# orting/image-feature-extraction

Hardware: AMD Instinct MI355X
Metric: Mvoxels/sec Hessian+eig, 512^3 fp32 3-scale (higher is better)
Workload: dtype f32 storage / f64 line recurrences

## Files before the change

### image-feature-extraction_amd/csrc/ife_capi.hip

```cpp
#include "../../include/ife_hip.h"

#include <hip/hip_runtime.h>

#include <algorithm>
#include <cmath>
#include <cstdarg>
#include <cstdio>
#include <cstdlib>
#include <cstring>
#include <map>
#include <new>
#include <string>
#include <tuple>
#include <type_traits>
#include <vector>

#include "feature_kernels.hpp"
#include "iir_types.hpp"
#include "stats_kernels.hpp"
#include "distance_kernels.hpp"
#include "dense_kernels.hpp"
#include "dense_plan.hpp"
#include "labels_kernels.hpp"
#include "deflate_kernels.hpp"
#include "resample_kernels.hpp"
#include "bspline_kernels.hpp"
#define IFE_IIR_NS iir_exact
#define IFE_IIR_FMA 0
#include "iir_kernels.inc"
#undef IFE_IIR_NS
#undef IFE_IIR_FMA
#define IFE_IIR_NS iir_fma
#define IFE_IIR_FMA 1
#include "iir_kernels.inc"
#undef IFE_IIR_NS
#undef IFE_IIR_FMA

using namespace ife;

namespace {

#define IFE_IIR_KERNELS(NS)                                                                      \
  struct NS##_kernels {                                                                          \
    template <int K> static constexpr auto contig = NS::iir_contig_kernel<K>;                    \
    template <int K> static constexpr auto strided1 = NS::iir_strided1_kernel<K>;                \
    template <int K, bool PAIRED, bool BWD> static constexpr auto strided = NS::iir_strided_kernel<K, PAIRED, BWD>; \
    template <int K, int S, typename TI, typename TM> static constexpr auto sweep_z = NS::iir_sweep_z_kernel<K, S, TI, TM>; \
    template <int K> static constexpr auto zslab_causal = NS::zslab_causal_kernel<K>;            \
    template <int K> static constexpr auto zslab_anti = NS::zslab_anti_kernel<K>;                \
    template <int K> static constexpr auto zslab_causal3 = NS::zslab_causal3_kernel<K>;          \
    template <int K> static constexpr auto zslab_anti3 = NS::zslab_anti3_kernel<K>;              \
    template <int K, int DIR> static constexpr auto zslab_fused = NS::zslab_fused_kernel<K, DIR>; \
    template <int K> static constexpr auto zslab_combine = NS::zslab_combine_kernel<K>;          \
  }
IFE_IIR_KERNELS(iir_exact);
IFE_IIR_KERNELS(iir_fma);
#undef IFE_IIR_KERNELS
template <typename F>
void with_iir_kernels(int fma, F &&f) {
  if (fma) f(iir_fma_kernels{});
  else f(iir_exact_kernels{});
}

template <int V0, int... Vs, typename F>
void with_const(int v, F &&f) {
  if constexpr (sizeof...(Vs) == 0) f(std::integral_constant<int, V0>{});
  else if (v == V0) f(std::integral_constant<int, V0>{});
  else with_const<Vs...>(v, f);
}

enum KernelKind {
  KK_IIR_Z = 0,
  KK_IIR_X,
  KK_IIR_Y,
  KK_ZSLAB_SWEEP,
  KK_ZSLAB_COMBINE,
  KK_FEATURES,
  KK_EIG_BATCH,
  KK_DIVIDE,
  KK_MASK,
  KK_PREP,
  KK_SORT_HIST,
  KK_SORT_SCAN,
  KK_SORT_SCATTER,
  KK_GATHER,
  KK_EDGES,
  KK_HIST,
  KK_EDT_X,
  KK_EDT_Y,
  KK_EDT_Z,
  KK_EDT_REDUCE,
  KK_DENSE_CODE,
  KK_DENSE_XY,
  KK_DENSE_Z,
  KK_JET,
  KK_COUNT
};
static_assert(KK_COUNT <= IFE_MAX_KERNEL_KINDS, "ife_get_kernel_times callers size their arrays by IFE_MAX_KERNEL_KINDS");
const char *kKindNames[KK_COUNT] = {"iir_z", "iir_x", "iir_y", "zslab_sweep", "zslab_combine", "features", "eig_batch",
                                    "divide", "mask_f64", "prep", "sort_hist", "sort_scan",
                                    "sort_scatter", "gather", "edges", "dense_histogram", "edt_x", "edt_y",
                                    "edt_z", "edt_reduce", "dense_code", "dense_box_xy", "dense_box_z", "jet_features"};

struct DevBuf {
  void *p = nullptr;
  size_t cap = 0;
  DevBuf() = default;
  DevBuf(DevBuf &&o) noexcept : p(std::exchange(o.p, nullptr)), cap(std::exchange(o.cap, 0)) {}
  DevBuf &operator=(DevBuf &&o) noexcept { std::swap(p, o.p); std::swap(cap, o.cap); return *this; }
  ~DevBuf() { (void)reset(); }
  hipError_t reset() {
    cap = 0;
    return p ? hipFree(std::exchange(p, nullptr)) : hipSuccess;
  }
  hipError_t grow(size_t bytes) {
    hipError_t e = reset();
    if (e == hipSuccess && (e = hipMalloc(&p, bytes)) == hipSuccess) cap = bytes;
    else p = nullptr;
    return e;
  }
};
constexpr int IFE_MAX_SLOTS = 3;

struct ProfRec {
  int kind;
  hipEvent_t a, b;
};

thread_local std::string g_create_error;

}

struct ife_ctx {
  int device = 0;
  hipStream_t stream = nullptr;
  std::string err;
  int trig_mode = 2;
  int dscale_mode = 0;
  int profile = 0;
  int zchunk = 64;
  int iir_block = 0;
  int iir_fma = 0;
  int iir_ckpt = 2;
  int fused_divide = 1;
  int const_lines = 1;
  int feat_ring = 1;
  int z_sweep = 1;
  int differential = 0;
  std::map<std::tuple<double, double, int64_t>, uint32_t> const_flags;
  DevBuf fld[IFE_MAX_SLOTS][4];
  DevBuf pre[2];
  DevBuf ck_y[IIR_MAX_JOBS];
  DevBuf zs_rec;
  DevBuf st_img, st_mask, st_aux, st_out;
  DevBuf edt_g, edt_i, edt_d2, edt_part;
  DevBuf dn_centres, dn_ws, dn_feat;
  int dense_scratch_mb = 0;
  struct DenseStream {
    bool open = false;
    DevBuf codes;
    DevBuf centres;
    DevBuf ws;
    DevBuf planar;
    DevBuf rows[2];
    hipEvent_t done[2] = {nullptr, nullptr};
    hipStream_t copy = nullptr;
    std::vector<DenseBlock> blocks;
    size_t next = 0, counted = 0;
    DenseGeom g;
    const uint8_t *flag = nullptr;
    const uint32_t *seg_base = nullptr;
    int ncol = 0, nb = 0, values = 0, cg = 0, bg = 0;
    int64_t n_rois = 0, ld = 0;
  } ds;
  DevBuf dj_ws;
  DevBuf sc_out;
  std::vector<hipEvent_t> sc_done;
  hipStream_t sc_copy = nullptr;
  size_t sc_scale_bytes = 0;
  int sc_layout = IFE_INTERLEAVED;
  DevBuf df_ws, df_out;
  DevBuf rs_tab;
  std::vector<ResampleEntry> rs_host;
  hipEvent_t rs_up = nullptr;
  DevBuf bs_coef, bs_tab;
  std::vector<double> bs_host;
  hipEvent_t bs_up = nullptr;
  std::vector<ProfRec> prof;
  std::vector<hipEvent_t> ev_pool;
  double acc_ms[KK_COUNT] = {0};
  int64_t acc_n[KK_COUNT] = {0};
};

namespace {

void dense_stream_release(ife_ctx *ctx);

int fail(ife_ctx *ctx, int code, const char *fmt, ...) {
  char buf[512];
// ... 231 lines not shown
    const double s2 = dscale_mode == 1 ? s1 * s1 : s1;
    d.m1[a] = -0.5 * s1;
    d.p1[a] = 0.5 * s1;
    d.a2[a] = 1.0 * s2;
    d.b2[a] = -2.0 * s2;
    d.c2[a] = 1.0 * s2;
  }
  return d;
}

IirGeom geom_for_axis(const ife_volume_desc *v, int axis) {
  IirGeom g;
  g.in_w = 0; g.in_group = 0; g.in_nz = 0;
  const int64_t nx = v->nx, ny = v->ny, nz = v->nz;
  if (axis == 2) {
    g.n = nz; g.nlines = nx * ny; g.sstride = nx * ny; g.inner = nx * ny; g.outer = 0;
  } else if (axis == 1) {
    g.n = ny; g.nlines = nx * nz; g.sstride = nx; g.inner = nx; g.outer = nx * ny;
  } else {
    g.n = nx; g.nlines = ny * nz; g.sstride = 1; g.inner = 1; g.outer = nx;
  }
  return g;
}

size_t ck_pairs(int64_t n, int K) { return (size_t)((n + K - 1) / K); }

int ensure_ck(ife_ctx *ctx, const ife_volume_desc *v, int njobs) {
  const int K = 8;
  size_t need_y = 0;
  for (int a = 0; a < 3; ++a) {
    IirGeom g = geom_for_axis(v, a);
    const size_t np = ck_pairs(g.n, K);
    need_y = std::max(need_y, np * 4 * (size_t)g.nlines * sizeof(double));
  }
  for (int j = 0; j < njobs; ++j) {
    int rc = ensure(ctx, ctx->ck_y[j], need_y);
    if (rc) return rc;
  }
  return IFE_OK;
}

int ensure_slots(ife_ctx *ctx, const ife_volume_desc *v, int nslots) {
  const size_t nb = (size_t)(v->nx * v->ny * v->nz) * sizeof(float);
  for (int s = 0; s < nslots; ++s)
    for (int i = 0; i < 4; ++i) {
      int rc = ensure(ctx, ctx->fld[s][i], nb);
      if (rc) return rc;
    }
  return IFE_OK;
}

struct ZSweepSrc {
  const void *img, *msk;
  int img_dtype, msk_dtype;
  float *tc, *cf;
  int nf;
  bool write_src;
};
int launch_iir(ife_ctx *ctx, const ife_volume_desc *v, int axis, int njobs,
               const float *const *in, float *const *out, const double *sigma,
               int in_y_chunks = 1, const int *order = nullptr ,
               const float *const *in2 = nullptr, const ZSweepSrc *zs = nullptr) {
  if (njobs < 1 || njobs > IIR_MAX_JOBS) return fail(ctx, IFE_E_ARG, "bad job count %d", njobs);
  IirGeom g = geom_for_axis(v, axis);
  if (in_y_chunks > 1) {
    if (axis != 0) return fail(ctx, IFE_E_ARG, "Y-chunked input is only read by the x pass");
    if (v->ny % in_y_chunks || (v->ny / in_y_chunks) % 64)
      return fail(ctx, IFE_E_SIZE, "Y-chunked input needs ny/chunks to be a multiple of 64");
    g.in_w = in_y_chunks;
    g.in_group = v->ny / in_y_chunks;
    g.in_nz = v->nz;
  }
  if ((int64_t)2 * 16 * g.sstride * 4 >= (int64_t)1 << 31 ||
      g.outer * 4 >= (int64_t)1 << 32 || g.nlines * 8 * 3 >= (int64_t)1 << 32)
    return fail(ctx, IFE_E_SIZE, "volume too large for the 32-bit offsets of the line kernels");
  if (in2 && (axis == 0 || 2 * njobs > IIR_MAX_JOBS || ctx->iir_ckpt != 2))
    return fail(ctx, IFE_E_ARG, "the paired form runs on the strided axes with at most %d jobs", IIR_MAX_JOBS / 2);
  if (zs && (axis != 2 || in2 || order || ctx->iir_ckpt != 2 || zs->nf < 1 || zs->nf > 2 || njobs % zs->nf ||
             njobs / zs->nf > IFE_MAX_SLOTS || !zs->img || !zs->tc || (zs->nf == 2 && (!zs->msk || !zs->cf))))
    return fail(ctx, IFE_E_ARG, "the shared sweep runs the Z pass of up to %d scales with pair checkpoints", IFE_MAX_SLOTS);
  int rc = ensure_ck(ctx, v, in2 ? 2 * njobs : njobs);
  if (rc) return rc;
  if (zs && (rc = ensure(ctx, ctx->zs_rec, (size_t)zs->nf * (size_t)g.nlines * sizeof(uint32_t)))) return rc;
  uint32_t any_const = 0;
  const double sp = axis == 0 ? v->sx : axis == 1 ? v->sy : v->sz;
  IirJobs jobs;
  memset(&jobs, 0, sizeof jobs);
  for (int j = 0; j < njobs; ++j) {
    if (!in[j] || !out[j] || in[j] == out[j]) return fail(ctx, IFE_E_ARG, "bad job buffers");
    if ((reinterpret_cast<uintptr_t>(in[j]) | reinterpret_cast<uintptr_t>(out[j])) % 4)
      return fail(ctx, IFE_E_ARG, "field pointers must be aligned to 4 bytes");
    jobs.j[j].in = in[j];
    jobs.j[j].out = out[j];
    jobs.j[j].ck_y = (double *)ctx->ck_y[j].p;
    if (in2) {
      if (!in2[j] || in2[j] == out[j] || reinterpret_cast<uintptr_t>(in2[j]) % 4)
        return fail(ctx, IFE_E_ARG, "bad denominator buffer");
      jobs.j[j].in2 = in2[j];
      jobs.j[j].ck_y2 = (double *)ctx->ck_y[njobs + j].p;
    }
    if (gauss_coeffs_order(sigma[j], sp, order ? order[j] : 0, &jobs.j[j].c))
      return fail(ctx, IFE_E_ARG, "spacing is suspiciously small");
    jobs.j[j].const_lines = 0;
    if (ctx->const_lines && !ctx->iir_fma && (!order || order[j] == 0)) {
      const int64_t len = axis == 0 ? v->nx : axis == 1 ? v->ny : v->nz;
      const std::tuple<double, double, int64_t> key(sigma[j], sp, len);
      auto it = ctx->const_flags.find(key);
      if (it == ctx->const_flags.end()) {
        if (ctx->const_flags.size() > 256) ctx->const_flags.clear();
        it = ctx->const_flags.emplace(key, const_line_flags(jobs.j[j].c, len)).first;
      }
      jobs.j[j].const_lines = it->second;
    }
    any_const |= jobs.j[j].const_lines;
    if (zs) jobs.j[j].line_rec = (const uint32_t *)ctx->zs_rec.p + (size_t)(j % zs->nf) * (size_t)g.nlines;
  }
  g.njobs = njobs;
  g.ngroups = (int32_t)((g.nlines + (in2 ? 127 : 255)) / (in2 ? 128 : 256));
  const dim3 grid((unsigned)((g.ngroups + 7) / 8 * 8 * njobs), 1, 1);
  const int sblock = ctx->iir_block ? ctx->iir_block : 12;
  if (zs) {
    ProfScope pz(ctx, KK_PREP);
    ZSweepArgs za;
    za.img = zs->img; za.msk = zs->msk; za.tc = zs->tc; za.cf = zs->cf;
    za.rec = (uint32_t *)ctx->zs_rec.p;
    za.nf = zs->nf; za.write_src = zs->write_src ? 1 : 0; za.track = any_const ? 1 : 0;
    IirGeom gs = g;
    gs.njobs = zs->nf;
    const dim3 sgrid((unsigned)((gs.ngroups + 7) / 8 * 8 * zs->nf), 1, 1);
    with_iir_kernels(ctx->iir_fma, [&](auto ks) {
      using KS = decltype(ks);
      with_const<8, 10, 12, 16>(sblock, [&](auto K) {
        with_const<1, 2, 3>(njobs / zs->nf, [&](auto S) {
          auto launch = [&](auto ti, auto tm) {
            hipLaunchKernelGGL((KS::template sweep_z<decltype(K)::value, decltype(S)::value, decltype(ti), decltype(tm)>),
                               sgrid, dim3(256), 0, ctx->stream, jobs, gs, za);
          };
          auto with_mask = [&](auto ti) {
            if (zs->msk && zs->msk_dtype == IFE_U16) launch(ti, uint16_t{});
            else launch(ti, uint8_t{});
          };
          if (zs->img_dtype == IFE_F32) with_mask(float{});
          else with_mask(int16_t{});
        });
      });
    });
    IFE_HIP(ctx, hipGetLastError());
  }
  ProfScope ps(ctx, axis == 2 ? KK_IIR_Z : axis == 1 ? KK_IIR_Y : KK_IIR_X);
  with_iir_kernels(ctx->iir_fma, [&](auto ks) {
    using KS = decltype(ks);
    auto launch = [&](auto kernel) { hipLaunchKernelGGL(kernel, grid, dim3(256), 0, ctx->stream, jobs, g); };
    if (zs)
      with_const<8, 10, 12, 16>(sblock, [&](auto K) { launch(KS::template strided<decltype(K)::value, false, true>); });
    else if (in2)
      with_const<8, 10, 12, 16>(sblock, [&](auto K) { launch(KS::template strided<decltype(K)::value, true, false>); });
    else if (axis == 0)
      with_const<8, 16>(ctx->iir_block, [&](auto K) { launch(KS::template contig<decltype(K)::value>); });
    else if (ctx->iir_ckpt == 1)
      with_const<8, 16>(ctx->iir_block, [&](auto K) { launch(KS::template strided1<decltype(K)::value>); });
    else
      with_const<8, 10, 12, 16>(sblock, [&](auto K) { launch(KS::template strided<decltype(K)::value, false, false>); });
  });
  IFE_HIP(ctx, hipGetLastError());
  return IFE_OK;
}

#ifndef IFE_ZSLAB_K
#define IFE_ZSLAB_K 12
#endif
constexpr int ZSLAB_K = IFE_ZSLAB_K;
int64_t zslab_pairs(int64_t n) { return ((n + ZSLAB_K - 1) / ZSLAB_K + 1) / 2; }
size_t zslab_ck_bytes(const ife_volume_desc *v) {
  const size_t L = (size_t)(v->nx * v->ny);
  return (size_t)zslab_pairs(v->nz) * 4 * L * 2 * sizeof(double);
}
int launch_zslab(ife_ctx *ctx, int phase, int njobs, const float *const *in, float *const *out,
                 const ife_volume_desc *v, int64_t line0, int64_t nlines, const double *sigmas,
                 int has_lo, int has_hi, const void *state_in, void *state_out, void *const *ck,
                 const int *orders = nullptr) {
  if (njobs < 1 || njobs > IIR_MAX_JOBS) return fail(ctx, IFE_E_ARG, "bad job count %d", njobs);
  for (int j = 0; orders && j < njobs; ++j)
    if (orders[j] < 0 || orders[j] > 2)
      return fail(ctx, IFE_E_ARG, "the order of the recursive Gaussian must be 0, 1 or 2");
  const int64_t L = v->nx * v->ny, n = v->nz;
  if (line0 < 0 || nlines < 1 || line0 + nlines > L)
    return fail(ctx, IFE_E_ARG, "line range [%lld, %lld) outside the %lld lines of the slab",
                (long long)line0, (long long)(line0 + nlines), (long long)L);
  if (n < 4) return fail(ctx, IFE_E_SIZE, "a Z-slab needs at least 4 planes (got %lld)", (long long)n);
  if ((int64_t)2 * ZSLAB_K * L * 4 >= (int64_t)1 << 31 || L * 8 * 3 >= (int64_t)1 << 32)
    return fail(ctx, IFE_E_SIZE, "slab too large for the 32-bit offsets of the line kernels");
  if (!in || !sigmas || !ck) return fail(ctx, IFE_E_ARG, "null pointer");
  const bool need_in = (phase == 0 || phase == 3) ? has_lo != 0 : (phase == 1 || phase == 4) ? has_hi != 0 : false;
  if ((phase != 2 && !state_out) || (need_in && !state_in)) return fail(ctx, IFE_E_ARG, "null state buffer");
  if ((reinterpret_cast<uintptr_t>(state_in) | reinterpret_cast<uintptr_t>(state_out)) % 8)
    return fail(ctx, IFE_E_ARG, "state buffers must be aligned to 8 bytes");
  const int64_t np = zslab_pairs(n);
  ZSlabJobs jobs, jobs3;
  memset(&jobs, 0, sizeof jobs);
  memset(&jobs3, 0, sizeof jobs3);
  int n1 = 0, n3 = 0, left3 = 0;
  for (int j = 0; j < njobs; ++j) {
    if (left3 == 0 && phase < 2 && orders && j + 2 < njobs && in[j] == in[j + 1] && in[j] == in[j + 2] &&
        sigmas[j] == sigmas[j + 1] && sigmas[j] == sigmas[j + 2] && orders[j] == 0 && orders[j + 1] == 1 &&
        orders[j + 2] == 2)
      left3 = 3;
    ZSlabJob &J = left3 > 0 ? jobs3.j[3 * n3 + (3 - left3)] : jobs.j[n1++];
    if (left3 > 0 && --left3 == 0) ++n3;
    if (!in[j] || !ck[j] || (phase >= 2 && (!out || !out[j] || out[j] == in[j])))
      return fail(ctx, IFE_E_ARG, "bad job buffers");
    if (reinterpret_cast<uintptr_t>(ck[j]) % 8 || reinterpret_cast<uintptr_t>(in[j]) % 4)
      return fail(ctx, IFE_E_ARG, "job buffers are misaligned");
    J.in = in[j] + line0;
    J.out = phase >= 2 ? out[j] + line0 : nullptr;
    double *cy = (double *)ck[j];
    double *ay = cy + np * 4 * L;
    J.cy = cy + line0; J.ay = ay + line0;
    const size_t rec = (size_t)nlines * IFE_Z_STATE_BYTES;
    if (state_in) J.sin_y = (const double *)((const char *)state_in + (size_t)j * rec);
    if (state_out) J.sout_y = (double *)((char *)state_out + (size_t)j * rec);
    if (!(sigmas[j] > 0.0) || gauss_coeffs_order(sigmas[j], v->sz, orders ? orders[j] : 0, &J.c))
      return fail(ctx, IFE_E_ARG, "bad sigma or spacing");
  }
  for (int t = 0; t < n3; ++t)
    for (int k = 1; k < 3; ++k)
      if (memcmp(&jobs3.j[3 * t].c.D1, &jobs3.j[3 * t + k].c.D1, 4 * sizeof(double)))
        return fail(ctx, IFE_E_STATE, "the feedback coefficients of one sigma differ between the orders");
  ZSlabGeom g;
  g.n = n; g.nlines = nlines; g.sstride = L; g.ck_stride = L;
  g.has_lo = has_lo ? 1 : 0; g.has_hi = has_hi ? 1 : 0;
  g.ngroups = (int32_t)((nlines + 255) / 256);
  ProfScope ps(ctx, phase >= 2 ? KK_ZSLAB_COMBINE : KK_ZSLAB_SWEEP);
  with_iir_kernels(ctx->iir_fma, [&](auto ks) {
    using KS = decltype(ks);
    auto launch = [&](auto kernel, const ZSlabJobs &js, int nj) {
      if (nj == 0) return;
      g.njobs = nj;
      const dim3 grid((unsigned)((g.ngroups + 7) / 8 * 8 * nj), 1, 1);
      hipLaunchKernelGGL(kernel, grid, dim3(256), 0, ctx->stream, js, g);
    };
    if (phase == 0) {
      launch(KS::template zslab_causal3<ZSLAB_K>, jobs3, n3);
      launch(KS::template zslab_causal<ZSLAB_K>, jobs, n1);
    } else if (phase == 1) {
      launch(KS::template zslab_anti3<ZSLAB_K>, jobs3, n3);
      launch(KS::template zslab_anti<ZSLAB_K>, jobs, n1);
    } else if (phase == 3) launch(KS::template zslab_fused<ZSLAB_K, 0>, jobs, n1);
    else if (phase == 4) launch(KS::template zslab_fused<ZSLAB_K, 1>, jobs, n1);
    else launch(KS::template zslab_combine<ZSLAB_K>, jobs, n1);
  });
  IFE_HIP(ctx, hipGetLastError());
  return IFE_OK;
}

template <typename TI, typename TM>
int launch_prep(ife_ctx *ctx, const TI *img, const TM *msk, float *tc, float *cf, int64_t n,
                PrepGeom pg = PrepGeom{0, 0, 0, 0, 0}) {
  ProfScope ps(ctx, KK_PREP);
  const uintptr_t al = reinterpret_cast<uintptr_t>(img) % (4 * sizeof(TI)) |
                       reinterpret_cast<uintptr_t>(msk) % (4 * sizeof(TM)) |
                       reinterpret_cast<uintptr_t>(tc) % 16 | reinterpret_cast<uintptr_t>(cf) % 16;
  const bool vec = al == 0 && (pg.chunks <= 1 || pg.nx % 4 == 0);
  const int64_t n4 = vec ? n / 4 : 0;
  if (n4 > 0) {
    const unsigned blocks = (unsigned)std::min<int64_t>((n4 + 255) / 256, 0x7fffffff);
    hipLaunchKernelGGL((prep_kernel_vec4<TI, TM>), dim3(blocks), dim3(256), 0, ctx->stream, img,
                       msk, tc, cf, n4, pg);
    IFE_HIP(ctx, hipGetLastError());
  }
  if (n4 * 4 < n) {
    const int64_t rest = n - n4 * 4;
    const unsigned blocks = (unsigned)std::min<int64_t>((rest + 255) / 256, 8192);
    hipLaunchKernelGGL((prep_kernel_scalar<TI, TM>), dim3(blocks), dim3(256), 0, ctx->stream,
                       img, msk, tc, cf, n4 * 4, n, pg);
    IFE_HIP(ctx, hipGetLastError());
  }
  return IFE_OK;
}

int smooth_group(ife_ctx *ctx, const float *src_num, const float *src_den,
                 const ife_volume_desc *v, const double *sigmas, int nscales, const ZSweepSrc *zs = nullptr) {
  const int nf = src_den ? 2 : 1;
  const float *in[IIR_MAX_JOBS];
  float *out[IIR_MAX_JOBS];
  double sg[IIR_MAX_JOBS];
  int nj = 0;
  for (int k = 0; k < nscales; ++k)
    for (int f = 0; f < nf; ++f) sg[nj++] = sigmas[k];
  int rc = ensure_slots(ctx, v, nscales);
  if (rc) return rc;
  auto fill = [&](int src_idx, int dst_idx, bool from_source) {
    int j = 0;
    for (int k = 0; k < nscales; ++k)
      for (int f = 0; f < nf; ++f, ++j) {
        in[j] = from_source ? (f == 0 ? src_num : src_den)
                            : (const float *)ctx->fld[k][2 * f + src_idx].p;
        out[j] = (float *)ctx->fld[k][2 * f + dst_idx].p;
      }
  };
  fill(0, 0, true);
  rc = launch_iir(ctx, v, 2, nj, in, out, sg, 1, nullptr, nullptr, zs);
  fill(0, 1, false);
  if (!rc) rc = launch_iir(ctx, v, 0, nj, in, out, sg);
  if (nf == 2 && ctx->fused_divide && ctx->iir_ckpt == 2) {
    const float *n1[IIR_MAX_JOBS], *d1[IIR_MAX_JOBS];
    float *o1[IIR_MAX_JOBS];
    double s1[IIR_MAX_JOBS];
    for (int k = 0; k < nscales; ++k) {
      n1[k] = (const float *)ctx->fld[k][1].p;
      d1[k] = (const float *)ctx->fld[k][3].p;
      o1[k] = (float *)ctx->fld[k][0].p;
      s1[k] = sigmas[k];
    }
    if (!rc) rc = launch_iir(ctx, v, 1, nscales, n1, o1, s1, 1, nullptr, d1);
    return rc;
// ... 743 lines not shown
```

### image-feature-extraction_amd/csrc/iir_kernels.inc

```
#include <hip/hip_runtime.h>
#include <stdint.h>

#include <hip/hip_runtime.h>
#include <stdint.h>

#include <stddef.h>

#include <type_traits>

#include "iir_types.hpp"

#if IFE_IIR_FMA
#define IFE_MADD(a, b, acc) fma((a), (b), (acc))
#else
#define IFE_MADD(a, b, acc) ((a) * (b) + (acc))
#endif

namespace ife {
namespace IFE_IIR_NS {




struct IirCoefMain {
// ... 170 lines not shown
__device__ __forceinline__ float buf_ld_as_f32<uint16_t>(rsrc_t r, uint32_t voff, uint32_t soff) {
  return (float)(uint16_t)__builtin_amdgcn_raw_buffer_load_b16(r, voff, soff, 0);
}
template <>
__device__ __forceinline__ float buf_ld_as_f32<int16_t>(rsrc_t r, uint32_t voff, uint32_t soff) {
  return (float)(int16_t)__builtin_amdgcn_raw_buffer_load_b16(r, voff, soff, 0);
}

__device__ __forceinline__ bool const_line_response(uint32_t bits, uint32_t flags, float &resp) {
  resp = __builtin_bit_cast(float, bits);
  if (bits == 0u) return (flags & 1u) != 0;
  if (bits == 0x3f800000u) return (flags & 2u) != 0;
  if (bits == 0x80000000u) {
    if (flags & 8u) resp = 0.0f;
    return (flags & 12u) != 0;
  }
  return false;
}
__device__ __forceinline__ bool same_bits(float a, float b) {
  return __builtin_bit_cast(uint32_t, a) == __builtin_bit_cast(uint32_t, b);
}


struct SrcF32 {
  const float *p;
  struct At { rsrc_t a; };
  __device__ __forceinline__ At at(int64_t u) const { return At{IFE_IN_RSRC(p + u)}; }
  __device__ __forceinline__ At at(int64_t u, uint32_t range) const { return At{make_rsrc_range(p + u, range)}; }
#if defined(IFE_DIAG_BYTE_LOADS)
  __device__ __forceinline__ float ld(const At &b, uint32_t v, uint32_t s) const {
    constexpr uint32_t E = IFE_DIAG_BYTE_LOADS == 1 ? 4u : 1u;
    return (float)(uint8_t)__builtin_amdgcn_raw_buffer_load_b8(b.a, v * E, s * E, 0);
  }
  __device__ __forceinline__ float ld_last(const At &b, uint32_t v, uint32_t s) const { return ld(b, v, s); }
#else
  __device__ __forceinline__ float ld(const At &b, uint32_t v, uint32_t s) const {
    return buf_ld_f32(b.a, v * 4u, s * 4u);
  }
  __device__ __forceinline__ float ld_last(const At &b, uint32_t v, uint32_t s) const {
    return buf_ld_last_f32(b.a, v * 4u, s * 4u);
  }
#endif
};

struct Checkpoint {
  double *y;
};

__device__ __forceinline__ void ck_store(const Checkpoint &ck, int64_t pair, int64_t nl,
                                         int64_t Lw, uint32_t lane, const CausalState &s) {
  const rsrc_t ry = IFE_CK_RSRC(ck.y + (pair * 4) * nl + Lw);
  const uint32_t sy = (uint32_t)nl * 8u;
  ck_st_f64(ry, lane * 8u, 0u, s.y1);
  ck_st_f64(ry, lane * 8u, sy, s.y2);
  ck_st_f64(ry, lane * 8u, 2u * sy, s.y3);
  ck_st_f64(ry, lane * 8u, 3u * sy, s.y4);
}
__device__ __forceinline__ void ck_load(const Checkpoint &ck, int64_t pair, int64_t nl,
                                        int64_t Lw, uint32_t lane, CausalState &s) {
  const rsrc_t ry = IFE_CK_RSRC(ck.y + (pair * 4) * nl + Lw);
  const uint32_t sy = (uint32_t)nl * 8u;
  s.y1 = ck_ld_f64(ry, lane * 8u, 0u);
  s.y2 = ck_ld_f64(ry, lane * 8u, sy);
  s.y3 = ck_ld_f64(ry, lane * 8u, 2u * sy);
  s.y4 = ck_ld_f64(ry, lane * 8u, 3u * sy);
}

__device__ __forceinline__ void opaque_state(CausalState &s) {
  asm volatile("" : "+v"(s.y1), "+v"(s.y2), "+v"(s.y3), "+v"(s.y4));
}

template <int K, bool STORE>
__device__ __forceinline__ void causal_run(CausalState &s, const float (&x)[K], double (&cz)[K],
                                           const IirCoef &c, int64_t i0, int64_t n, bool edge) {
  if (!edge) {
#pragma unroll
    for (int j = 0; j < K; ++j) {
      const double y = causal_step(s, (double)x[j], c);
      if (STORE) cz[j] = y;
    }
  } else {
#pragma unroll
    for (int j = 0; j < K; ++j)
      if (i0 + j < n) {
        const double y = causal_step_edge(s, (double)x[j], c, i0 + j);
        if (STORE) cz[j] = y;
      }
  }
}
#ifndef IFE_IIR_LDS_CZ
#define IFE_IIR_LDS_CZ 1
#endif
template <int K>
__device__ __forceinline__ void causal_run_park(CausalState &s, const float (&x)[K], double *col,
                                                const IirCoef &c, int64_t i0, int64_t n, bool edge) {
  if (!edge) {
#pragma unroll
    for (int j = 0; j < K; ++j) col[j * 64] = causal_step(s, (double)x[j], c);
  } else {
#pragma unroll
    for (int j = 0; j < K; ++j)
      if (i0 + j < n) col[j * 64] = causal_step_edge(s, (double)x[j], c, i0 + j);
  }
}
template <int K>
__device__ __forceinline__ void causal_unpark(double (&cz)[K], const double *col) {
#pragma unroll
  for (int j = 0; j < K; ++j) cz[j] = col[j * 64];
}
template <int K>
__device__ __forceinline__ void anti_run_parked(AntiState &a, float (&x)[K], const double *col,
                                                const IirCoef &c, int64_t i0, int64_t n, bool edge) {
  if (!edge) {
#pragma unroll
    for (int j = K - 1; j >= 0; --j) {
      const double y = anti_step(a, (double)x[j], c);
      x[j] = (float)(col[j * 64] + y);
    }
  } else {
#pragma unroll
    for (int j = K - 1; j >= 0; --j)
      if (i0 + j < n) {
        const double y = anti_step_edge(a, (double)x[j], c, i0 + j, n);
        x[j] = (float)(col[j * 64] + y);
      }
  }
}

template <int K>
__device__ __forceinline__ void anti_run(AntiState &a, float (&x)[K], const double (&cz)[K],
                                         const IirCoef &c, int64_t i0, int64_t n, bool edge) {
  if (!edge) {
#pragma unroll
    for (int j = K - 1; j >= 0; --j) {
      const double y = anti_step(a, (double)x[j], c);
      x[j] = (float)(cz[j] + y);
    }
  } else {
#pragma unroll
    for (int j = K - 1; j >= 0; --j)
      if (i0 + j < n) {
        const double y = anti_step_edge(a, (double)x[j], c, i0 + j, n);
        x[j] = (float)(cz[j] + y);
      }
  }
}

__device__ __forceinline__ void lds_workgroup_sync() {
  asm volatile("s_waitcnt lgkmcnt(0)\n\ts_barrier" ::: "memory");
}
#ifndef IFE_IIR_FENCE
#define IFE_IIR_FENCE 2
#endif
template <int K, bool PAIRED = false, bool BWD = false>
__global__ __launch_bounds__(256, K <= 10 ? 4 : (IFE_IIR_LDS_CZ && K <= 12 ? 3 : 1)) void iir_strided_kernel(IirJobs jobs, IirGeom g) {
  static_assert(!(PAIRED && BWD), "the backward-only form is the plain form of the first axis pass");
  const IirBlock blk = iir_block_of(g, blockIdx.x);
  if (!blk.live) return;
  const IirJob &J = jobs.j[blk.job];
  const uint32_t lane = threadIdx.x & 63u;
  const uint32_t wave_id = __builtin_amdgcn_readfirstlane(threadIdx.x >> 6);
  const bool is_den = PAIRED && wave_id >= 2u;
  const uint32_t out_range = (wave_id >> 1) - 1u;
  const SrcF32 src{is_den ? J.in2 : J.in};
  float *__restrict__ out = J.out;
  const IirCoefMain c = main_coefs(J.c);
  const Checkpoint ck{is_den ? J.ck_y2 : J.ck_y};
  int64_t Lw = PAIRED ? uniform64((int64_t)blk.group * 128 + (int64_t)(wave_id & 1u) * 64)
                      : uniform64((int64_t)blk.group * blockDim.x + (int64_t)(threadIdx.x & ~63u));
  const bool wave_dead = Lw >= g.nlines;
  if (!PAIRED && wave_dead) return;
  if (wave_dead) Lw = 0;
  const int64_t n = g.n, st = g.sstride, nl = g.nlines;
  int64_t L = Lw + lane;
  if (L >= nl) L = nl - 1;
  const uint32_t cl = (uint32_t)(L - Lw);
  const int64_t base = (L % g.inner) + (L / g.inner) * g.outer;
  const int64_t wbase = uniform64(base);
  const uint32_t voff = (uint32_t)(base - wbase);
  const uint32_t sst = (uint32_t)st;
  const int nb = (int)((n + K - 1) / K);
  const int np = (nb + 1) / 2;
#if IFE_IIR_LDS_CZ
  __shared__ double park[4][2 * K][64];
  double *col = &park[threadIdx.x >> 6][0][lane];
#else
#error "the strided kernel parks the causal values of a pair in LDS"
#endif

  bool fwd_const = true;
  float fwd_ref = 0.0f;
  CausalState turn;
  turn.x1 = turn.x2 = turn.x3 = 0.0;
  turn.y1 = turn.y2 = turn.y3 = turn.y4 = 0.0;
  if constexpr (!BWD) {
    float a0[K], a1[K], b0[K], b1[K];
    CausalState s;
    const int nfp = np - 1;
    auto load_pair_f = [&](int p, float (&u)[K], float (&v)[K]) {
      const auto B = src.at(wbase + (int64_t)(2 * p * K) * st, mask_lt(p, nfp));
#pragma unroll
      for (int j = 0; j < K; ++j) u[j] = src.ld(B, voff, (uint32_t)j * sst);
#pragma unroll
      for (int j = 0; j < K; ++j) v[j] = src.ld(B, voff, (uint32_t)(K + j) * sst);
    };
    auto track = [&](const float (&x)[K]) {
      if constexpr (!PAIRED) {
        if (J.const_lines) {
#pragma unroll
          for (int j = 0; j < K; ++j) fwd_const = fwd_const && same_bits(x[j], fwd_ref);
        }
      }
    };
    auto run_pair = [&](int p, const float (&u)[K], const float (&v)[K]) {
#pragma unroll
      for (int j = 0; j < 3; ++j) causal_step(s, (double)u[j], c);
      ck_store(ck, p, nl, Lw, cl, s);
#pragma unroll
      for (int j = 3; j < K; ++j) causal_step(s, (double)u[j], c);
      track(u);
#pragma unroll
      for (int j = 0; j < K; ++j) causal_step(s, (double)v[j], c);
      track(v);
    };
    if (nfp > 0) {
      load_pair_f(0, a0, a1);
      load_pair_f(1, b0, b1);
      {
        const double e0 = (double)a0[0];
        fwd_ref = a0[0];
        s.x1 = s.x2 = s.x3 = e0;
        s.y1 = s.y2 = s.y3 = s.y4 = e0;
        {
          const IirCoef ce = edge_coefs(blk.job);
#pragma unroll
          for (int j = 0; j < K; ++j) causal_step_edge(s, (double)a0[j], ce, j);
        }
        track(a0);
#pragma unroll
        for (int j = 0; j < K; ++j) causal_step(s, (double)a1[j], c);
        track(a1);
      }
      load_pair_f(2, a0, a1);
      int p = 1;
      for (; p + 1 < nfp; p += 2) {
        run_pair(p, b0, b1);
        load_pair_f(p + 2, b0, b1);
        run_pair(p + 1, a0, a1);
        load_pair_f(p + 3, a0, a1);
      }
      if (p < nfp) run_pair(p, b0, b1);
      turn = s;
    }
  } else {
    if (np > 1) {
      ck_load(ck, np - 1, nl, Lw, cl, turn);
      const auto B = src.at(wbase + ((int64_t)(2 * (np - 1) * K) - 3) * st);
      turn.x3 = (double)src.ld(B, voff, 0u);
      turn.x2 = (double)src.ld(B, voff, sst);
      turn.x1 = (double)src.ld(B, voff, 2u * sst);
      if (J.const_lines) fwd_ref = __builtin_bit_cast(float, J.line_rec[L]);
    }
  }

  {
    float xa[K], xb[K];
    float na[K], nb2[K];
    AntiState a;
    auto load_pair = [&](int p, float (&pa)[K], float (&pb)[K], bool clampn) {
      const int64_t i0 = (int64_t)(2 * p * K);
      const auto B = src.at(wbase + i0 * st);
      if (!clampn) {
#pragma unroll
        for (int j = 0; j < K; ++j) pa[j] = src.ld_last(B, voff, (uint32_t)j * sst);
#pragma unroll
        for (int j = 0; j < K; ++j) pb[j] = src.ld_last(B, voff, (uint32_t)(K + j) * sst);
      } else {
        const uint32_t lastj = (uint32_t)(n - 1 - i0);
#pragma unroll
        for (int j = 0; j < K; ++j)
          pa[j] = src.ld_last(B, voff, ((uint32_t)j < lastj ? (uint32_t)j : lastj) * sst);
#pragma unroll
        for (int j = 0; j < K; ++j)
          pb[j] = src.ld_last(B, voff, ((uint32_t)(K + j) < lastj ? (uint32_t)(K + j) : lastj) * sst);
      }
    };
    CausalState sc, sn;
    sc.y1 = sc.y2 = sc.y3 = sc.y4 = 0.0;
    sn = sc;
    load_pair(np - 1, xa, xb, true);
    bool wave_const = false;
    float cval = 0.0f;
    if (!PAIRED && J.const_lines) {
      const float first = xa[0];
      bool cst = np == 1 || (fwd_const && same_bits(fwd_ref, first));
#pragma unroll
      for (int j = 0; j < K; ++j) cst = cst && same_bits(xa[j], first) && same_bits(xb[j], first);
      cst = const_line_response(__builtin_bit_cast(uint32_t, first), J.const_lines, cval) && cst;
      wave_const = __builtin_amdgcn_ballot_w64(!cst) == 0;
    }
    if (wave_const && !PAIRED) {
      for (int p = np - 1; p >= 0; --p) {
        const int64_t i0 = (int64_t)(2 * p * K);
        const rsrc_t ro = IFE_OUT_RSRC(out + wbase + i0 * st);
#pragma unroll
        for (int j = 0; j < 2 * K; ++j)
          if (i0 + j < n) buf_st_out_f32(ro, voff * 4u, (uint32_t)j * sst * 4u, cval);
      }
      return;
    }
    {
      const double xN = (double)xb[K - 1];
      a.x1 = a.x2 = a.x3 = a.x4 = xN;
      a.y1 = a.y2 = a.y3 = a.y4 = xN;
    }
    float *fx = PAIRED ? reinterpret_cast<float *>(&park[is_den ? wave_id : wave_id + 2u][0][0]) + lane : nullptr;
    auto quotient = [&](int64_t i0, int64_t i1) {
      bool ones = true;
#pragma unroll
      for (int j = 0; j < K; ++j)
        ones = ones && (fx[j * 64] == 1.0f || i0 + j >= n) && (fx[(K + j) * 64] == 1.0f || i1 + j >= n);
      if (__builtin_amdgcn_ballot_w64(!ones) != 0) {
#pragma unroll
        for (int j = 0; j < K; ++j) {
          const float da = fx[j * 64], db = fx[(K + j) * 64];
          xa[j] = da != 0.0f ? xa[j] / da : 3.402823466e+38f;
          xb[j] = db != 0.0f ? xb[j] / db : 3.402823466e+38f;
        }
      }
    };
    auto rotate = [&]() {
#pragma unroll
      for (int j = 0; j < K; ++j) { xa[j] = na[j]; xb[j] = nb2[j]; }
      sc.y1 = sn.y1; sc.y2 = sn.y2; sc.y3 = sn.y3; sc.y4 = sn.y4;
    };

    auto steady_iter = [&](int p) {
      const int64_t i0 = (int64_t)(2 * p * K);
      CausalState s;
      s.y1 = sc.y1; s.y2 = sc.y2; s.y3 = sc.y3; s.y4 = sc.y4;
      s.x1 = (double)xa[2]; s.x2 = (double)xa[1]; s.x3 = (double)xa[0];
      col[0] = sc.y3; col[64] = sc.y2; col[128] = sc.y1;
      __builtin_amdgcn_sched_barrier(0);
#pragma unroll
      for (int j = 3; j < K; ++j) {
        col[j * 64] = causal_step(s, (double)xa[j], c);
        if (j % IFE_IIR_FENCE == IFE_IIR_FENCE - 1) __builtin_amdgcn_sched_barrier(0);
      }
      __builtin_amdgcn_sched_barrier(0);
#pragma unroll
      for (int j = 0; j < K; ++j) {
        col[(K + j) * 64] = causal_step(s, (double)xb[j], c);
        if (j % IFE_IIR_FENCE == IFE_IIR_FENCE - 1) __builtin_amdgcn_sched_barrier(0);
      }
      __builtin_amdgcn_sched_barrier(0);
      load_pair(p - 1, na, nb2, false);
      ck_load(ck, p - 1, nl, Lw, cl, sn);
      __builtin_amdgcn_sched_barrier(0);
#pragma unroll
      for (int j = K - 1; j >= 0; --j) {
        xb[j] = (float)(col[(K + j) * 64] + anti_step(a, (double)xb[j], c));
        if (j % IFE_IIR_FENCE == 0) __builtin_amdgcn_sched_barrier(0);
      }
      __builtin_amdgcn_sched_barrier(0);
#pragma unroll
      for (int j = K - 1; j >= 0; --j) {
        xa[j] = (float)(col[j * 64] + anti_step(a, (double)xa[j], c));
        if (j % IFE_IIR_FENCE == 0) __builtin_amdgcn_sched_barrier(0);
      }
      __builtin_amdgcn_sched_barrier(0);
      if constexpr (PAIRED) {
        if (is_den) {
#pragma unroll
          for (int j = 0; j < K; ++j) { fx[j * 64] = xa[j]; fx[(K + j) * 64] = xb[j]; }
        }
        lds_workgroup_sync();
        if (!is_den) quotient(i0, i0 + K);
      }
      const rsrc_t ro = PAIRED ? IFE_OUT_RSRC_RANGE(out + wbase + i0 * st, out_range) : IFE_OUT_RSRC(out + wbase + i0 * st);
#pragma unroll
      for (int j = 0; j < K; ++j) buf_st_out_f32(ro, voff * 4u, (uint32_t)(K + j) * sst * 4u, xb[j]);
#pragma unroll
      for (int j = 0; j < K; ++j) buf_st_out_f32(ro, voff * 4u, (uint32_t)j * sst * 4u, xa[j]);
      if constexpr (PAIRED) lds_workgroup_sync();
      rotate();
    };

    auto general_iter = [&](int p, auto turn_tag) {
      constexpr bool TURN = decltype(turn_tag)::value;
      const int64_t i0 = (int64_t)(2 * p * K), i1 = i0 + K;
      const IirCoef ce = edge_coefs(blk.job);
      if (p > 0) {
        load_pair(p - 1, na, nb2, false);
        if (p > 1) ck_load(ck, p - 1, nl, Lw, cl, sn);
      }
      const bool head = p == 0;
      const bool tail = i1 + K + 4 > n;
      const rsrc_t ro = PAIRED ? IFE_OUT_RSRC_RANGE(out + wbase + i0 * st, out_range) : IFE_OUT_RSRC(out + wbase + i0 * st);
      const bool edge = head || (i0 + K + 4 > n);
      CausalState s;
      if (head || TURN) {
        if (head) {
          const double x0 = (double)xa[0];
          s.x1 = s.x2 = s.x3 = x0;
          s.y1 = s.y2 = s.y3 = s.y4 = x0;
        } else {
          s = turn;
        }
        causal_run_park<K>(s, xa, col, ce, i0, n, edge);
      } else {
        s.y1 = sc.y1; s.y2 = sc.y2; s.y3 = sc.y3; s.y4 = sc.y4;
        s.x1 = (double)xa[2]; s.x2 = (double)xa[1]; s.x3 = (double)xa[0];
        col[0] = sc.y3; col[64] = sc.y2; col[128] = sc.y1;
#pragma unroll
        for (int j = 3; j < K; ++j) col[j * 64] = causal_step(s, (double)xa[j], ce);
      }
      if (i1 < n) {
        causal_run_park<K>(s, xb, col + K * 64, ce, i1, n, tail);
        anti_run_parked<K>(a, xb, col + K * 64, ce, i1, n, tail);
      }
      anti_run_parked<K>(a, xa, col, ce, i0, n, edge);
      if constexpr (PAIRED) {
        if (is_den) {
#pragma unroll
          for (int j = 0; j < K; ++j) { fx[j * 64] = xa[j]; fx[(K + j) * 64] = xb[j]; }
        }
        lds_workgroup_sync();
        if (!is_den) quotient(i0, i1);
      }
      if (i1 < n) {
#pragma unroll
        for (int j = 0; j < K; ++j)
          if (!tail || i1 + j < n) buf_st_out_f32(ro, voff * 4u, (uint32_t)(K + j) * sst * 4u, xb[j]);
      }
#pragma unroll
      for (int j = 0; j < K; ++j)
        if (!edge || i0 + j < n) buf_st_out_f32(ro, voff * 4u, (uint32_t)j * sst * 4u, xa[j]);
      if constexpr (PAIRED) lds_workgroup_sync();
      rotate();
    };

    const int p_hi = (int)((n - 4) / (2 * K)) - 1;
    general_iter(np - 1, std::true_type{});
    int p = np - 2;
    while (p >= 0) {
      if (p >= 2 && p <= p_hi) {
        __builtin_amdgcn_s_waitcnt(0x0F70);
        do {
          steady_iter(p);
          --p;
        } while (p >= 2);
      } else {
        general_iter(p, std::false_type{});
        --p;
      }
    }
  }
}

template <int K>
__global__ __launch_bounds__(256) void iir_strided1_kernel(IirJobs jobs, IirGeom g) {
  const IirBlock blk = iir_block_of(g, blockIdx.x);
  if (!blk.live) return;
  const IirJob &J = jobs.j[blk.job];
  const SrcF32 src{J.in};
  float *__restrict__ out = J.out;
  const IirCoef c = J.c;
  const Checkpoint ck{J.ck_y};
  const uint32_t lane = threadIdx.x & 63u;
  const int64_t Lw =
      uniform64((int64_t)blk.group * blockDim.x + (int64_t)(threadIdx.x & ~63u));
  if (Lw >= g.nlines) return;
  const int64_t n = g.n, st = g.sstride, nl = g.nlines;
  int64_t L = Lw + lane;
  const bool live = L < nl;
  if (!live) L = nl - 1;
  const int64_t base = (L % g.inner) + (L / g.inner) * g.outer;
  const int64_t wbase = uniform64(base);
  const uint32_t voff = (uint32_t)(base - wbase);
  const uint32_t sst = (uint32_t)st;
  const int64_t nb = (n + K - 1) / K;

  {
    float xb[K], xn[K];
    CausalState s;
    if (nb > 1) {
      const auto B = src.at(wbase);
#pragma unroll
      for (int j = 0; j < K; ++j) xb[j] = src.ld(B, voff, (uint32_t)j * sst);
    }
    for (int64_t b = 0; b + 1 < nb; ++b) {
      const int64_t i0 = b * K;
      if (b + 2 < nb) {
        const auto B = src.at(wbase + (i0 + K) * st);
#pragma unroll
        for (int j = 0; j < K; ++j) xn[j] = src.ld(B, voff, (uint32_t)j * sst);
      }
      if (b > 0) {
#pragma unroll
        for (int j = 0; j < K; ++j) causal_step(s, (double)xb[j], c);
      } else {
        const double x0 = (double)xb[0];
        s.x1 = s.x2 = s.x3 = x0;
        s.y1 = s.y2 = s.y3 = s.y4 = x0;
#pragma unroll
        for (int j = 0; j < K; ++j) causal_step_edge(s, (double)xb[j], c, j);
      }
      if (live) ck_store(ck, b + 1, nl, Lw, lane, s);
#pragma unroll
      for (int j = 0; j < K; ++j) xb[j] = xn[j];
    }
  }

  {
    float xa[K], na[K];
    float h1 = 0.f, h2 = 0.f, h3 = 0.f, nh1 = 0.f, nh2 = 0.f, nh3 = 0.f;
    AntiState a;
    CausalState sc, sn;
    sc.y1 = sc.y2 = sc.y3 = sc.y4 = 0.0;
    sn = sc;
    auto load_hist = [&](int64_t b, float &q1, float &q2, float &q3) {
      const auto B = src.at(wbase + (b * K - 3) * st);
      q3 = src.ld(B, voff, 0u);
      q2 = src.ld(B, voff, sst);
      q1 = src.ld(B, voff, 2u * sst);
    };
    {
      const int64_t i0 = (nb - 1) * K;
      const auto B = src.at(wbase + i0 * st);
      const uint32_t lastj = (uint32_t)(n - 1 - i0);
#pragma unroll
      for (int j = 0; j < K; ++j)
        xa[j] = src.ld(B, voff, ((uint32_t)j < lastj ? (uint32_t)j : lastj) * sst);
      if (nb > 1) {
        load_hist(nb - 1, h1, h2, h3);
        ck_load(ck, nb - 1, nl, Lw, live ? lane : 0u, sc);
      }
      const double xN = (double)xa[K - 1];
      a.x1 = a.x2 = a.x3 = a.x4 = xN;
      a.y1 = a.y2 = a.y3 = a.y4 = xN;
    }
    for (int64_t b = nb - 1; b >= 0; --b) {
      const int64_t i0 = b * K;
      if (b > 0) {
        const auto B = src.at(wbase + (i0 - K) * st);
#pragma unroll
        for (int j = 0; j < K; ++j) na[j] = src.ld(B, voff, (uint32_t)j * sst);
        if (b > 1) {
          load_hist(b - 1, nh1, nh2, nh3);
          ck_load(ck, b - 1, nl, Lw, live ? lane : 0u, sn);
        }
      }
      CausalState s;
      if (b > 0) {
        s.y1 = sc.y1; s.y2 = sc.y2; s.y3 = sc.y3; s.y4 = sc.y4;
        s.x1 = (double)h1; s.x2 = (double)h2; s.x3 = (double)h3;
      } else {
        const double x0 = (double)xa[0];
        s.x1 = s.x2 = s.x3 = x0;
        s.y1 = s.y2 = s.y3 = s.y4 = x0;
      }
      const bool edge = (b == 0) || (i0 + K + 4 > n);
      double cz[K];
      causal_run<K, true>(s, xa, cz, c, i0, n, edge);
      anti_run<K>(a, xa, cz, c, i0, n, edge);
      if (live) {
        const rsrc_t ro = IFE_OUT_RSRC(out + wbase + i0 * st);
#pragma unroll
        for (int j = 0; j < K; ++j)
          if (!edge || i0 + j < n) buf_st_out_f32(ro, voff * 4u, (uint32_t)j * sst * 4u, xa[j]);
      }
#pragma unroll
      for (int j = 0; j < K; ++j) xa[j] = na[j];
      h1 = nh1; h2 = nh2; h3 = nh3;
      sc.y1 = sn.y1; sc.y2 = sn.y2; sc.y3 = sn.y3; sc.y4 = sn.y4;
    }
  }
}

template <typename T>
__device__ __forceinline__ uint32_t buf_ld_raw(rsrc_t r, uint32_t voff, uint32_t soff);
template <>
__device__ __forceinline__ uint32_t buf_ld_raw<float>(rsrc_t r, uint32_t voff, uint32_t soff) {
  return __builtin_amdgcn_raw_buffer_load_b32(r, voff, soff, 0);
}
template <>
__device__ __forceinline__ uint32_t buf_ld_raw<int16_t>(rsrc_t r, uint32_t voff, uint32_t soff) {
  return (uint32_t)(uint16_t)__builtin_amdgcn_raw_buffer_load_b16(r, voff, soff, 0);
}
template <>
__device__ __forceinline__ uint32_t buf_ld_raw<uint16_t>(rsrc_t r, uint32_t voff, uint32_t soff) {
  return (uint32_t)(uint16_t)__builtin_amdgcn_raw_buffer_load_b16(r, voff, soff, 0);
}
template <>
__device__ __forceinline__ uint32_t buf_ld_raw<uint8_t>(rsrc_t r, uint32_t voff, uint32_t soff) {
  return (uint32_t)(uint8_t)__builtin_amdgcn_raw_buffer_load_b8(r, voff, soff, 0);
}
template <typename T>
__device__ __forceinline__ float raw_as_f32(uint32_t r) {
  if constexpr (std::is_same<T, float>::value) return __builtin_bit_cast(float, r);
  else if constexpr (std::is_same<T, int16_t>::value) return (float)(int16_t)(uint16_t)r;
  else return (float)r;
}
struct SweepY {
  double y1, y2, y3, y4;
};
template <typename C>
__device__ __forceinline__ void sweep_step(SweepY &s, double x1, double x2, double x3, double xin, const C &c) {
  const double a = IFE_MADD(x3, c.N3, IFE_MADD(x2, c.N2, IFE_MADD(x1, c.N1, xin * c.N0)));
// ... 1200 lines not shown
```

Measured before the change: 48610.

## Split z-axis backward IIR pass into dedicated kernel with prefetched checkpoints

Replaces the BWD template variant of the strided IIR kernel with a separate kernel for the z-axis backward pass after a slab forward sweep. The new kernel recomputes each causal segment from stored checkpoints, parks it in LDS, and runs the anti-causal recurrence. It prefetches the next pair's samples and checkpoint state while the current pair is processed, and places explicit scheduling barriers around the steps. It also adds an early-out for constant lines. The aim is to overlap global loads with the serial double-precision recurrences and to simplify the plain strided kernel, at the cost of more code and register pressure.

```diff
diff --git a/image-feature-extraction_amd/csrc/ife_capi.hip b/image-feature-extraction_amd/csrc/ife_capi.hip
--- a/image-feature-extraction_amd/csrc/ife_capi.hip
+++ b/image-feature-extraction_amd/csrc/ife_capi.hip
@@ -44,7 +44,8 @@
   struct NS##_kernels {                                                                          \
     template <int K> static constexpr auto contig = NS::iir_contig_kernel<K>;                    \
     template <int K> static constexpr auto strided1 = NS::iir_strided1_kernel<K>;                \
-    template <int K, bool PAIRED, bool BWD> static constexpr auto strided = NS::iir_strided_kernel<K, PAIRED, BWD>; \
+    template <int K, bool PAIRED> static constexpr auto strided = NS::iir_strided_kernel<K, PAIRED>; \
+    template <int K> static constexpr auto bwd_z = NS::iir_bwd_z_kernel<K>;                      \
     template <int K, int S, typename TI, typename TM> static constexpr auto sweep_z = NS::iir_sweep_z_kernel<K, S, TI, TM>; \
     template <int K> static constexpr auto zslab_causal = NS::zslab_causal_kernel<K>;            \
     template <int K> static constexpr auto zslab_anti = NS::zslab_anti_kernel<K>;                \
@@ -582,15 +583,15 @@
     using KS = decltype(ks);
     auto launch = [&](auto kernel) { hipLaunchKernelGGL(kernel, grid, dim3(256), 0, ctx->stream, jobs, g); };
     if (zs)
-      with_const<8, 10, 12, 16>(sblock, [&](auto K) { launch(KS::template strided<decltype(K)::value, false, true>); });
+      with_const<8, 10, 12, 16>(sblock, [&](auto K) { launch(KS::template bwd_z<decltype(K)::value>); });
     else if (in2)
-      with_const<8, 10, 12, 16>(sblock, [&](auto K) { launch(KS::template strided<decltype(K)::value, true, false>); });
+      with_const<8, 10, 12, 16>(sblock, [&](auto K) { launch(KS::template strided<decltype(K)::value, true>); });
     else if (axis == 0)
       with_const<8, 16>(ctx->iir_block, [&](auto K) { launch(KS::template contig<decltype(K)::value>); });
     else if (ctx->iir_ckpt == 1)
       with_const<8, 16>(ctx->iir_block, [&](auto K) { launch(KS::template strided1<decltype(K)::value>); });
     else
-      with_const<8, 10, 12, 16>(sblock, [&](auto K) { launch(KS::template strided<decltype(K)::value, false, false>); });
+      with_const<8, 10, 12, 16>(sblock, [&](auto K) { launch(KS::template strided<decltype(K)::value, false>); });
   });
   IFE_HIP(ctx, hipGetLastError());
   return IFE_OK;
diff --git a/image-feature-extraction_amd/csrc/iir_kernels.inc b/image-feature-extraction_amd/csrc/iir_kernels.inc
--- a/image-feature-extraction_amd/csrc/iir_kernels.inc
+++ b/image-feature-extraction_amd/csrc/iir_kernels.inc
@@ -346,9 +346,8 @@
 #ifndef IFE_IIR_FENCE
 #define IFE_IIR_FENCE 2
 #endif
-template <int K, bool PAIRED = false, bool BWD = false>
+template <int K, bool PAIRED = false>
 __global__ __launch_bounds__(256, K <= 10 ? 4 : (IFE_IIR_LDS_CZ && K <= 12 ? 3 : 1)) void iir_strided_kernel(IirJobs jobs, IirGeom g) {
-  static_assert(!(PAIRED && BWD), "the backward-only form is the plain form of the first axis pass");
   const IirBlock blk = iir_block_of(g, blockIdx.x);
   if (!blk.live) return;
   const IirJob &J = jobs.j[blk.job];
@@ -387,7 +386,7 @@
   CausalState turn;
   turn.x1 = turn.x2 = turn.x3 = 0.0;
   turn.y1 = turn.y2 = turn.y3 = turn.y4 = 0.0;
-  if constexpr (!BWD) {
+  {
     float a0[K], a1[K], b0[K], b1[K];
     CausalState s;
     const int nfp = np - 1;
@@ -445,15 +444,6 @@
       }
       if (p < nfp) run_pair(p, b0, b1);
       turn = s;
-    }
-  } else {
-    if (np > 1) {
-      ck_load(ck, np - 1, nl, Lw, cl, turn);
-      const auto B = src.at(wbase + ((int64_t)(2 * (np - 1) * K) - 3) * st);
-      turn.x3 = (double)src.ld(B, voff, 0u);
-      turn.x2 = (double)src.ld(B, voff, sst);
-      turn.x1 = (double)src.ld(B, voff, 2u * sst);
-      if (J.const_lines) fwd_ref = __builtin_bit_cast(float, J.line_rec[L]);
     }
   }
 
@@ -649,6 +639,191 @@
         --p;
       }
     }
+  }
+}
+
+__device__ __forceinline__ void ck_load(const Checkpoint &ck, int64_t pair, int64_t nl, int64_t Lw,
+                                        uint32_t lane, CausalState &s, uint32_t range) {
+#if defined(IFE_DIAG_NO_CK)
+  range = 0u;
+#endif
+  const rsrc_t ry = make_rsrc_range(ck.y + (pair * 4) * nl + Lw, range);
+  const uint32_t sy = (uint32_t)nl * 8u;
+  s.y1 = ck_ld_f64(ry, lane * 8u, 0u);
+  s.y2 = ck_ld_f64(ry, lane * 8u, sy);
+  s.y3 = ck_ld_f64(ry, lane * 8u, 2u * sy);
+  s.y4 = ck_ld_f64(ry, lane * 8u, 3u * sy);
+}
+template <int K>
+__global__ __launch_bounds__(256, K <= 10 ? 4 : (K <= 12 ? 3 : 1)) void iir_bwd_z_kernel(IirJobs jobs, IirGeom g) {
+  const IirBlock blk = iir_block_of(g, blockIdx.x);
+  if (!blk.live) return;
+  const IirJob &J = jobs.j[blk.job];
+  const uint32_t lane = threadIdx.x & 63u;
+  const int64_t Lw = uniform64((int64_t)blk.group * blockDim.x + (int64_t)(threadIdx.x & ~63u));
+  if (Lw >= g.nlines) return;
+  const SrcF32 src{J.in};
+  float *__restrict__ out = J.out;
+  const IirCoefMain c = main_coefs(J.c);
+  const Checkpoint ck{J.ck_y};
+  const int64_t n = g.n, nl = g.nlines;
+  int64_t L = Lw + lane;
+  if (L >= nl) L = nl - 1;
+  const uint32_t cl = (uint32_t)(L - Lw);
+  const uint32_t sst = (uint32_t)nl;
+  const int nb = (int)((n + K - 1) / K);
+  const int np = (nb + 1) / 2;
+  __shared__ double park[4][2 * K][64];
+  double *col = &park[threadIdx.x >> 6][0][lane];
+
+  float xa[K], xb[K];
+  float na[K], nb2[K];
+  AntiState a;
+  CausalState sc, sn;
+  auto request = [&](int q, float (&pa)[K], float (&pb)[K], CausalState &s, uint32_t range, uint32_t ck_range) {
+    const auto B = src.at(Lw + (int64_t)(2 * q * K) * nl, range);
+#pragma unroll
+    for (int j = 0; j < K; ++j) pa[j] = src.ld_last(B, cl, (uint32_t)j * sst);
+#pragma unroll
+    for (int j = 0; j < K; ++j) pb[j] = src.ld_last(B, cl, (uint32_t)(K + j) * sst);
+    ck_load(ck, q, nl, Lw, cl, s, ck_range);
+  };
+  auto rotate = [&]() {
+#pragma unroll
+    for (int j = 0; j < K; ++j) { xa[j] = na[j]; xb[j] = nb2[j]; }
+    sc.y1 = sn.y1; sc.y2 = sn.y2; sc.y3 = sn.y3; sc.y4 = sn.y4;
+  };
+
+  const int pl = np - 1;
+  const int64_t il = (int64_t)(2 * pl * K);
+  const uint32_t swept = mask_lt(0, pl);
+  float fwd_ref = 0.0f;
+  if (J.const_lines && pl > 0) fwd_ref = __builtin_bit_cast(float, J.line_rec[L]);
+  CausalState turn;
+  ck_load(ck, pl, nl, Lw, cl, turn, swept);
+  {
+    const int64_t r0 = pl > 0 ? il - 3 : 0;
+    const auto B = src.at(Lw + r0 * nl, swept);
+    turn.x3 = (double)src.ld(B, cl, 0u);
+    turn.x2 = (double)src.ld(B, cl, sst);
+    turn.x1 = (double)src.ld(B, cl, 2u * sst);
+  }
+  {
+    const auto B = src.at(Lw + il * nl);
+    const uint32_t lastj = (uint32_t)(n - 1 - il);
+#pragma unroll
+    for (int j = 0; j < K; ++j)
+      xa[j] = src.ld_last(B, cl, ((uint32_t)j < lastj ? (uint32_t)j : lastj) * sst);
+#pragma unroll
+    for (int j = 0; j < K; ++j)
+      xb[j] = src.ld_last(B, cl, ((uint32_t)(K + j) < lastj ? (uint32_t)(K + j) : lastj) * sst);
+  }
+  if (J.const_lines) {
+    float cval = 0.0f;
+    const float first = xa[0];
+    bool cst = pl == 0 || same_bits(fwd_ref, first);
+#pragma unroll
+    for (int j = 0; j < K; ++j) cst = cst && same_bits(xa[j], first) && same_bits(xb[j], first);
+    cst = const_line_response(__builtin_bit_cast(uint32_t, first), J.const_lines, cval) && cst;
+    if (__builtin_amdgcn_ballot_w64(!cst) == 0) {
+      for (int p = pl; p >= 0; --p) {
+        const int64_t i0 = (int64_t)(2 * p * K);
+        const rsrc_t ro = IFE_OUT_RSRC(out + Lw + i0 * nl);
+#pragma unroll
+        for (int j = 0; j < 2 * K; ++j)
+          if (i0 + j < n) buf_st_out_f32(ro, cl * 4u, (uint32_t)j * sst * 4u, cval);
+      }
+      return;
+    }
+  }
+  {
+    const double xN = (double)xb[K - 1];
+    a.x1 = a.x2 = a.x3 = a.x4 = xN;
+    a.y1 = a.y2 = a.y3 = a.y4 = xN;
+  }
+  {
+    const int64_t i1 = il + K;
+    const int q = pl > 0 ? pl - 1 : 0;
+    request(q, na, nb2, sn, swept, mask_lt(1, pl));
+    const IirCoef ce = edge_coefs(blk.job);
+    const bool head = pl == 0;
+    const bool edge = head || (il + K + 4 > n);
+    CausalState s;
+    if (head) {
+      const double x0 = (double)xa[0];
+      s.x1 = s.x2 = s.x3 = x0;
+      s.y1 = s.y2 = s.y3 = s.y4 = x0;
+    } else {
+      s = turn;
+    }
+    causal_run_park<K>(s, xa, col, ce, il, n, edge);
+    if (i1 < n) {
+      causal_run_park<K>(s, xb, col + K * 64, ce, i1, n, true);
+      anti_run_parked<K>(a, xb, col + K * 64, ce, i1, n, true);
+    }
+    anti_run_parked<K>(a, xa, col, ce, il, n, edge);
+    const rsrc_t ro = IFE_OUT_RSRC_RANGE(out + Lw + il * nl, ((uint32_t)(n - il) * sst - (uint32_t)Lw) * 4u);
+#pragma unroll
+    for (int j = 0; j < K; ++j) buf_st_out_f32(ro, (cl + (uint32_t)(K + j) * sst) * 4u, 0u, xb[j]);
+#pragma unroll
+    for (int j = 0; j < K; ++j) buf_st_out_f32(ro, (cl + (uint32_t)j * sst) * 4u, 0u, xa[j]);
+    rotate();
+  }
+
+  for (int p = pl - 1; p >= 0; --p) {
+    const int64_t i0 = (int64_t)(2 * p * K);
+    CausalState s;
+    if (p == 0) {
+      const IirCoef ce = edge_coefs(blk.job);
+      const double x0 = (double)xa[0];
+      s.x1 = s.x2 = s.x3 = x0;
+      s.y1 = s.y2 = s.y3 = s.y4 = x0;
+#pragma unroll
+      for (int j = 0; j < 4; ++j) col[j * 64] = causal_step_edge(s, (double)xa[j], ce, j);
+    } else {
+      s.y1 = sc.y1; s.y2 = sc.y2; s.y3 = sc.y3; s.y4 = sc.y4;
+      s.x1 = (double)xa[2]; s.x2 = (double)xa[1]; s.x3 = (double)xa[0];
+      col[0] = sc.y3; col[64] = sc.y2; col[128] = sc.y1;
+      col[3 * 64] = causal_step(s, (double)xa[3], c);
+    }
+    __builtin_amdgcn_sched_barrier(0);
+#pragma unroll
+    for (int j = 4; j < K; ++j) {
+      col[j * 64] = causal_step(s, (double)xa[j], c);
+      if (j % IFE_IIR_FENCE == IFE_IIR_FENCE - 1) __builtin_amdgcn_sched_barrier(0);
+    }
+    __builtin_amdgcn_sched_barrier(0);
+#pragma unroll
+    for (int j = 0; j < K; ++j) {
+      col[(K + j) * 64] = causal_step(s, (double)xb[j], c);
+      if (j % IFE_IIR_FENCE == IFE_IIR_FENCE - 1) __builtin_amdgcn_sched_barrier(0);
+    }
+    __builtin_amdgcn_sched_barrier(0);
+    request(p > 0 ? p - 1 : 0, na, nb2, sn, mask_lt(0, p), mask_lt(1, p));
+    __builtin_amdgcn_sched_barrier(0);
+    if (i0 + 2 * K + 4 > n) {
+      const IirCoef ce = edge_coefs(blk.job);
+      anti_run_parked<K>(a, xb, col + K * 64, ce, i0 + K, n, true);
+    } else {
+#pragma unroll
+      for (int j = K - 1; j >= 0; --j) {
+        xb[j] = (float)(col[(K + j) * 64] + anti_step(a, (double)xb[j], c));
+        if (j % IFE_IIR_FENCE == 0) __builtin_amdgcn_sched_barrier(0);
+      }
+    }
+    __builtin_amdgcn_sched_barrier(0);
+#pragma unroll
+    for (int j = K - 1; j >= 0; --j) {
+      xa[j] = (float)(col[j * 64] + anti_step(a, (double)xa[j], c));
+      if (j % IFE_IIR_FENCE == 0) __builtin_amdgcn_sched_barrier(0);
+    }
+    __builtin_amdgcn_sched_barrier(0);
+    const rsrc_t ro = IFE_OUT_RSRC(out + Lw + i0 * nl);
+#pragma unroll
+    for (int j = 0; j < K; ++j) buf_st_out_f32(ro, cl * 4u, (uint32_t)(K + j) * sst * 4u, xb[j]);
+#pragma unroll
+    for (int j = 0; j < K; ++j) buf_st_out_f32(ro, cl * 4u, (uint32_t)j * sst * 4u, xa[j]);
+    rotate();
   }
 }
 
```

After: 48740, median of 6. No clear change (+0.3%).
